# olegroshka/vae-channel-dynamics

Measured on AMD Instinct MI355X. Metric: images/sec SDXL-VAE train step @256x256 (tracking on), higher is better.
Workload: dtype f32

## Files before the change

### vae-channel-dynamics_amd/csrc/igemm.hip

```cpp
#include "bf16_frag.h"
#include <algorithm>
#include <stdlib.h>
#include <type_traits>

#include "launchers.h"

namespace {

struct LanePos {
  int lr, lh, trq, trp, trh;
};
__device__ __forceinline__ LanePos lane_pos(int lane) { return LanePos{lane & 31, lane >> 5, (lane & 15) >> 2, lane & 3, (lane >> 4) & 1}; }

struct F32 {
  typedef float elem;
  typedef f32x4 raw4;
  typedef f32x4 frag;
  typedef unsigned off_t;
  static constexpr int BK_ROWS = 32, BK_WGRAD = 32;
  static constexpr int KG = 8;
  static constexpr int PAD_K = 4, PAD_T = 4;
  static constexpr bool SETPRIO = true;
  static constexpr bool PAIR16 = false;
  static constexpr bool flag(int32_t) { return false; }
// ... 506 lines not shown
      if (XF != VAE_XF_NONE) {
        const bool ok = xb[i] >= 0;
        const int o = ok ? (xb[i] - b_lo) * BN + b4 * 4 : 0;
        v = xform4_tab<XF>(v, sS + o, sS + SS_HALF + o, ok);
      }
      P::put4(&sB[(bkq + BKR * i) * LDB + b4 * 4], v);
    }
  };
  typename P::frag fa[2][MI], fb[2][NI];
  auto fetch = [&](const elem* sA, const elem* sB, int kg, typename P::frag* a, typename P::frag* b) {
    P::template frags_tt<MI, NI>(a, b, sA, LDA, wm * TM, sB, LDB, wn * TN, kg, lp);
  };
  constexpr int NKG = BK / P::KG;
  auto compute = [&](const elem* sA, const elem* sB, int kg) {
    if (kg + 1 < NKG) fetch(sA, sB, kg + 1, fa[(kg + 1) & 1], fb[(kg + 1) & 1]);
    __builtin_amdgcn_sched_barrier(0);
    if (P::SETPRIO) __builtin_amdgcn_s_setprio(1);
    P::mma(acc, fa[kg & 1], fb[kg & 1]);
    if (P::SETPRIO) __builtin_amdgcn_s_setprio(0);
    __builtin_amdgcn_sched_barrier(0);
  };
  if (steps > 0) {
    load_regs(0);
    __syncthreads();
    store_lds(smem, smem + SA);
    if (steps > 1) load_regs(1);
    __syncthreads();
    for (int s = 0; s < steps; ++s) {
      const elem* cA = smem + (s & 1) * STAGE;
      const elem* cB = cA + SA;
      fetch(cA, cB, 0, fa[0], fb[0]);
      compute(cA, cB, 0);
      if (NKG == 4) compute(cA, cB, 1);
      if (s + 1 < steps) {
        elem* nA = smem + ((s + 1) & 1) * STAGE;
        store_lds(nA, nA + SA);
        if (s + 2 < steps) load_regs(s + 2);
      }
      compute(cA, cB, NKG / 2);
      if (NKG == 4) compute(cA, cB, 3);
      __syncthreads();
    }
  }

  const int64_t ld = (int64_t)g.taps * p.N;
  float* __restrict__ O = (p.nsplit == 1 ? p.out : p.partial + (int64_t)split * p.M * ld) + (int64_t)z * p.sOb;
#pragma unroll
  for (int ni = 0; ni < NI; ++ni) {
    const int col = n0 + wn * TN + ni * 32 + lr;
    if (col >= p.N) continue;
#pragma unroll
    for (int mi = 0; mi < MI; ++mi)
#pragma unroll
      for (int r = 0; r < 16; ++r) {
        const int row = m0 + wm * TM + mi * 32 + (r & 3) + 8 * (r >> 2) + 4 * lh;
        if (row < p.M) O[(int64_t)row * ld + (int64_t)tap * p.N + col] = p.alpha * acc[mi][ni][r];
      }
  }
  if (do_bias) {
    f32x4* red = reinterpret_cast<f32x4*>(smem);
    red[akq * AQ + a4] = bsum;
    __syncthreads();
    if (tid < AQ) {
      f32x4 t = {0.f, 0.f, 0.f, 0.f};
      for (int r = 0; r < AKR; ++r) t += red[r * AQ + tid];
#pragma unroll
      for (int e = 0; e < 4; ++e) {
        const int m = m0 + tid * 4 + e;
        if (m < p.M) p.bias_partial[(int64_t)split * p.M + m] = t[e];
      }
    }
  }
}

template <int BM, int BN, int WM, int WN, bool BKM, bool VEC, int XF>
__global__ __launch_bounds__(64 * WM * WN) void igemm_rows_kernel(vae_igemm_args p) { rows_body<F32, BM, BN, WM, WN, BKM, VEC, XF>(p); }
template <int BM, int BN, int WM, int WN, bool VEC, int XF>
__global__ __launch_bounds__(64 * WM * WN) void wgrad_kernel(vae_wgrad_args p) { wgrad_body<F32, BM, BN, WM, WN, VEC, XF>(p); }
template <int BM, int BN, int WM, int WN, bool BKM, int XF>
__global__ __launch_bounds__(64 * WM * WN) void igemm_rows_bf16_kernel(vae_igemm_args p) { rows_body<BF16, BM, BN, WM, WN, BKM, true, XF>(p); }
template <int BM, int BN, int WM, int WN, int XF>
__global__ __launch_bounds__(64 * WM * WN) void wgrad_bf16_kernel(vae_wgrad_args p) { wgrad_body<BF16, BM, BN, WM, WN, true, XF>(p); }

template <int KP>
__global__ __launch_bounds__(256) void reduce_splits_kernel(const float* __restrict__ partial, int nsplit, int64_t n, float* __restrict__ out,
                                                            int main_blocks, const float* __restrict__ partial2, int n2, float* __restrict__ out2) {
  constexpr int COLS = 256 / KP;
  __shared__ f32x4 red[KP > 1 ? 256 : 1];
  if ((int)blockIdx.x >= main_blocks) {
    const int i = ((int)blockIdx.x - main_blocks) * 256 + threadIdx.x;
    if (i < n2) {
      float s2 = 0.f;
      for (int k = 0; k < nsplit; ++k) s2 += partial2[(int64_t)k * n2 + i];
      out2[i] = s2;
    }
    return;
  }
  const int col = threadIdx.x % COLS, kp = threadIdx.x / COLS;
  const int64_t n4 = n >> 2;
  const int per = (nsplit + KP - 1) / KP;
  const int k0 = kp * per, k1 = min(nsplit, k0 + per);
  auto column = [&](int64_t i) {
    f32x4 s = {0.f, 0.f, 0.f, 0.f};
    const f32x4* p = reinterpret_cast<const f32x4*>(partial) + i;
    int k = k0;
    for (; k + 8 <= k1; k += 8) {
      f32x4 v[8];
#pragma unroll
      for (int j = 0; j < 8; ++j) v[j] = p[(int64_t)(k + j) * n4];
      s += ((v[0] + v[1]) + (v[2] + v[3])) + ((v[4] + v[5]) + (v[6] + v[7]));
    }
    for (; k < k1; ++k) s += p[(int64_t)k * n4];
    return s;
  };
  if (KP == 1) {
    for (int64_t i = (int64_t)blockIdx.x * 256 + threadIdx.x; i < n4; i += (int64_t)main_blocks * 256) reinterpret_cast<f32x4*>(out)[i] = column(i);
    return;
  }
  const int64_t i = (int64_t)blockIdx.x * COLS + col;
  f32x4 s = {0.f, 0.f, 0.f, 0.f};
  if (i < n4) s = column(i);
  red[threadIdx.x] = s;
  __syncthreads();
  if (kp == 0 && i < n4) {
#pragma unroll
    for (int j = 1; j < KP; ++j) s += red[j * COLS + col];
    reinterpret_cast<f32x4*>(out)[i] = s;
  }
}
__global__ void reduce_splits_scalar_kernel(const float* __restrict__ partial, int nsplit, int64_t n, float* __restrict__ out) {
  int64_t i = (int64_t)blockIdx.x * blockDim.x + threadIdx.x;
  const int64_t stride = (int64_t)gridDim.x * blockDim.x;
  for (; i < n; i += stride) {
    float s = 0.f;
    for (int k = 0; k < nsplit; ++k) s += partial[(int64_t)k * n + i];
    out[i] = s;
  }
}

template <int V>
using int_c = std::integral_constant<int, V>;
using std::false_type;
using std::true_type;

template <class Launch>
bool dispatch_xf(int xf, Launch launch) {
  switch (xf) {
    case VAE_XF_NONE: launch(int_c<VAE_XF_NONE>{}); return true;
    case VAE_XF_AFFINE: launch(int_c<VAE_XF_AFFINE>{}); return true;
    case VAE_XF_AFFINE_SILU: launch(int_c<VAE_XF_AFFINE_SILU>{}); return true;
    default: return false;
  }
}

template <bool BF, int BM, int BN, int WM, int WN>
int launch_rows_tile(const vae_igemm_args& a, bool bkm, bool vec, hipStream_t st) {
  const dim3 grid((unsigned)(((a.M + BM - 1) / BM) * ((a.N + BN - 1) / BN)), 1, (unsigned)a.batch), block(64 * WM * WN);
  auto go = [&](auto bkm_c, auto vec_c) {
    constexpr bool BKM = decltype(bkm_c)::value, VEC = decltype(vec_c)::value;
    auto launch = [&](auto xf) {
      if constexpr (BF) hipLaunchKernelGGL((igemm_rows_bf16_kernel<BM, BN, WM, WN, BKM, decltype(xf)::value>), grid, block, 0, st, a);
      else hipLaunchKernelGGL((igemm_rows_kernel<BM, BN, WM, WN, BKM, VEC, decltype(xf)::value>), grid, block, 0, st, a);
    };
    if constexpr (BKM) {
      if (a.xf != VAE_XF_NONE) { vae_set_error("igemm_rows: xf unsupported with n-contiguous weights"); return VAE_EINVAL; }
      launch(int_c<VAE_XF_NONE>{});
    } else if (!dispatch_xf(a.xf, launch)) {
      vae_set_error("igemm_rows: bad xf %d", a.xf);
      return VAE_EINVAL;
    }
    return 0;
  };
  if (BF || vec) return bkm ? go(true_type{}, true_type{}) : go(false_type{}, true_type{});
  if constexpr (!BF) return bkm ? go(true_type{}, false_type{}) : go(false_type{}, false_type{});
  return 0;
}
template <bool BF>
int launch_rows(const vae_igemm_args& a, bool bkm, bool vec, hipStream_t st) {
  return (a.N <= 32) ? launch_rows_tile<BF, 128, 32, 4, 1>(a, bkm, vec, st) : launch_rows_tile<BF, 128, 128, 4, 2>(a, bkm, vec, st);
}

template <bool BF, int BM, int BN, int WM, int WN>
int launch_wgrad_tile(const vae_wgrad_args& a, bool vec, hipStream_t st) {
  const dim3 grid((unsigned)(((a.M + BM - 1) / BM) * ((a.N + BN - 1) / BN)), (unsigned)(a.g.taps * a.nsplit), (unsigned)a.batch), block(64 * WM * WN);
  auto go = [&](auto vec_c) {
    auto launch = [&](auto xf) {
      if constexpr (BF) hipLaunchKernelGGL((wgrad_bf16_kernel<BM, BN, WM, WN, decltype(xf)::value>), grid, block, 0, st, a);
      else hipLaunchKernelGGL((wgrad_kernel<BM, BN, WM, WN, decltype(vec_c)::value, decltype(xf)::value>), grid, block, 0, st, a);
    };
    if (dispatch_xf(a.xf, launch)) return 0;
    vae_set_error("wgrad: bad xf %d", a.xf);
    return VAE_EINVAL;
  };
  if (BF || vec) return go(true_type{});
  if constexpr (!BF) return go(false_type{});
  return 0;
}
template <bool BF>
int launch_wgrad(const vae_wgrad_args& a, bool vec, hipStream_t st) {
  if (a.M <= 32) return launch_wgrad_tile<BF, 32, 128, 1, 4>(a, vec, st);
  if (a.N <= 32) return launch_wgrad_tile<BF, 128, 32, 4, 1>(a, vec, st);
  return launch_wgrad_tile<BF, 128, 128, 4, 2>(a, vec, st);
}

}

int launch_rows_f32(const vae_igemm_args& a, bool bkm, bool vec, hipStream_t st) { return launch_rows<false>(a, bkm, vec, st); }
int launch_rows_bf16(const vae_igemm_args& a, bool bkm, hipStream_t st) { return launch_rows<true>(a, bkm, true, st); }
int launch_wgrad_f32(const vae_wgrad_args& a, bool vec, hipStream_t st) { return launch_wgrad<false>(a, vec, st); }
int launch_wgrad_bf16(const vae_wgrad_args& a, hipStream_t st) { return launch_wgrad<true>(a, true, st); }

static int reduce_splits_impl(const float* partial, int32_t nsplit, int64_t n, float* out, const float* partial2, int32_t n2, float* out2,
                              hipStream_t st) {
  const int extra = partial2 ? (n2 + 255) / 256 : 0;
  if (n % 4 == 0 && aligned16(partial) && aligned16(out)) {
    const int64_t n4 = n / 4;
    if (nsplit >= 32) {
      const int64_t blocks = (n4 + 63) / 64;
      VAE_CHECK(blocks + extra < (1ll << 31), "reduce_splits: too many elements");
      hipLaunchKernelGGL(reduce_splits_kernel<4>, dim3((unsigned)(blocks + extra)), dim3(256), 0, st, partial, nsplit, n, out, (int)blocks, partial2, n2, out2);
    } else {
      const int64_t blocks = std::min<int64_t>((n4 + 255) / 256, 8192);
      hipLaunchKernelGGL(reduce_splits_kernel<1>, dim3((unsigned)(blocks + extra)), dim3(256), 0, st, partial, nsplit, n, out, (int)blocks, partial2, n2, out2);
    }
  } else {
    int blocks = (int)((n + 255) / 256);
    if (blocks > 4096) blocks = 4096;
    hipLaunchKernelGGL(reduce_splits_scalar_kernel, dim3(blocks), dim3(256), 0, st, partial, nsplit, n, out);
    if (partial2) hipLaunchKernelGGL(reduce_splits_scalar_kernel, dim3(extra), dim3(256), 0, st, partial2, nsplit, (int64_t)n2, out2);
  }
  return 0;
}
extern "C" int vae_reduce_splits(const float* partial, int32_t nsplit, int64_t n, float* out, void* stream) {
  VAE_CHECK(partial && out && nsplit > 0 && n > 0, "reduce_splits: bad args");
  if (int rc = reduce_splits_impl(partial, nsplit, n, out, nullptr, 0, nullptr, (hipStream_t)stream)) return rc;
  VAE_LAUNCH_CHECK("reduce_splits");
  return VAE_OK;
}
extern "C" int vae_reduce_splits2(const float* partial, int32_t nsplit, int64_t n, float* out, const float* partial2, int32_t n2, float* out2,
                                  void* stream) {
  VAE_CHECK(partial && out && partial2 && out2 && nsplit > 0 && n > 0 && n2 > 0, "reduce_splits2: bad args");
  if (int rc = reduce_splits_impl(partial, nsplit, n, out, partial2, n2, out2, (hipStream_t)stream)) return rc;
  VAE_LAUNCH_CHECK("reduce_splits2");
  return VAE_OK;
}
extern "C" int vae_wgrad_wino_reduce(const float* slab, int32_t nsplit, int32_t npos, int32_t Cin, int32_t Cout, float* scratch, float* dW,
                                     const float* bias_partial, float* db, void* stream) {
  VAE_CHECK(slab && dW && nsplit > 0 && Cin > 0 && Cout > 0 && Cin % 32 == 0 && Cout % 32 == 0, "wgrad_wino_reduce: bad args");
  VAE_CHECK(npos == 16 || npos == 9, "wgrad_wino_reduce: npos must be 16 (plain 3x3 layer) or 9 (upsampler convolution)");
  VAE_CHECK((bias_partial == nullptr) == (db == nullptr), "wgrad_wino_reduce: bias_partial and db go together");
  VAE_CHECK(nsplit == 1 || scratch != nullptr, "wgrad_wino_reduce: nsplit > 1 needs the [16*Cin*Cout] scratch buffer");
  hipStream_t st = (hipStream_t)stream;
  if (nsplit > 1) {
    if (int rc = reduce_splits_impl(slab, nsplit, (int64_t)npos * Cin * Cout, scratch, bias_partial, bias_partial ? Cout : 0, db, st)) return rc;
    VAE_LAUNCH_CHECK("reduce_splits");
    if (int rc = (npos == 9 ? launch_upwino_wgrad_reduce : launch_wino_wgrad_reduce)(scratch, 1, Cin, Cout, dW, nullptr, nullptr, st)) return rc;
  } else {
    if (int rc = (npos == 9 ? launch_upwino_wgrad_reduce : launch_wino_wgrad_reduce)(slab, 1, Cin, Cout, dW, bias_partial, db, st)) return rc;
  }
  VAE_LAUNCH_CHECK("wino_wgrad_reduce");
  return VAE_OK;
}
```

### vae-channel-dynamics_amd/csrc/launchers.h

```cpp
#pragma once
#include "common_host.h"

int launch_rows_f32(const vae_igemm_args& a, bool bkm, bool vec, hipStream_t st);
int launch_wgrad_f32(const vae_wgrad_args& a, bool vec, hipStream_t st);
int launch_rows_bf16(const vae_igemm_args& a, bool bkm, hipStream_t st);
int launch_wgrad_bf16(const vae_wgrad_args& a, hipStream_t st);

bool conv3_tile_eligible(const vae_igemm_args& a, bool vec, bool bkm);
int conv3_tile_gstat_chunks(const vae_igemm_args& a);
int launch_conv3_tile(const vae_igemm_args& a, bool bkm, hipStream_t st);
bool conv3_tile_bf16_packed(const vae_igemm_args& a);
int conv3_tile_bf16_gstat_chunks(const vae_igemm_args& a);
int launch_conv3_tile_bf16(const vae_igemm_args& a, bool bkm, hipStream_t st);
bool conv3_wide_bf16_eligible(const vae_igemm_args& a);
int conv3_wide_bf16_gstat_chunks(const vae_igemm_args& a);
int launch_conv3_wide_bf16(const vae_igemm_args& a, hipStream_t st);
bool conv3_wino_eligible(const vae_igemm_args& a);
int conv3_wino_nb();
int conv3_wino_gstat_chunks(const vae_igemm_args& a);
int conv3_wino_gnb_chunks(const vae_igemm_args& a);
int launch_wino_weights(const vae_igemm_args& a, float* U, hipStream_t st);
int launch_conv3_wino(const vae_igemm_args& a, const float* U, hipStream_t st);
bool conv3_wino4_eligible(const vae_igemm_args& a);
int conv3_wino4_gstat_chunks(const vae_igemm_args& a);
int conv3_wino4_gnb_chunks(const vae_igemm_args& a);
int launch_wino4_weights(const vae_igemm_args& a, float* U, hipStream_t st);
int launch_conv3_wino4(const vae_igemm_args& a, const float* U, hipStream_t st);
bool conv3_upwino_eligible(const vae_igemm_args& a);
int launch_upwino_weights(const vae_igemm_args& a, float* U, hipStream_t st);
int launch_conv3_upwino(const vae_igemm_args& a, const float* U, hipStream_t st);
bool conv1_bf16_eligible(const vae_igemm_args& a);
int launch_conv1_bf16(const vae_igemm_args& a, hipStream_t st);
bool conv_smallk_eligible(const vae_igemm_args& a);
int launch_conv_smallk(const vae_igemm_args& a, hipStream_t st);
bool conv_smalln_eligible(const vae_igemm_args& a);
int launch_conv_smalln(const vae_igemm_args& a, hipStream_t st);
bool conv_thin_bf16_eligible(const vae_igemm_args& a);
int launch_conv_thin_bf16(const vae_igemm_args& a, hipStream_t st);
bool conv_thinn_bf16_eligible(const vae_igemm_args& a);
int launch_conv_thinn_bf16(const vae_igemm_args& a, hipStream_t st);
int wgrad_smallk_kind(const vae_wgrad_args& a);
int wgrad_smallk_tiles(const vae_wgrad_args& a);
int launch_wgrad_smallk(const vae_wgrad_args& a, hipStream_t st);
bool wgrad_thin_bf16_eligible(const vae_wgrad_args& a, int kind);
int launch_wgrad_thin(const vae_wgrad_args& a, hipStream_t st);

bool wgrad3_tile_eligible(const vae_wgrad_args& a, bool vec);
int64_t wgrad3_tile_units(const vae_conv_geom& g);
int launch_wgrad3_tile(const vae_wgrad_args& a, hipStream_t st);
bool wgrad3_dma_bf16_operands(const vae_wgrad_args& a);
bool wgrad3_tile_bf16_eligible(const vae_wgrad_args& a, bool vec, bool dma);
int64_t wgrad3_tile_bf16_units(const vae_conv_geom& g);
int wgrad3_tile_bf16_columns(const vae_wgrad_args& a);
int launch_wgrad3_tile_bf16(const vae_wgrad_args& a, hipStream_t st);
int launch_wgrad3_dma_bf16(const vae_wgrad_args& a, hipStream_t st);
bool wgrad3_wino_eligible(const vae_wgrad_args& a);
int64_t wgrad3_wino_units(const vae_conv_geom& g);
int launch_wgrad3_wino(const vae_wgrad_args& a, hipStream_t st);
int launch_wino_wgrad_reduce(const float* slab, int nsplit, int N, int M, float* dW, const float* bpart, float* db, hipStream_t st);
bool wgrad3_upwino_eligible(const vae_wgrad_args& a);
int64_t wgrad3_upwino_units(const vae_conv_geom& g);
int launch_wgrad3_upwino(const vae_wgrad_args& a, hipStream_t st);
int launch_upwino_wgrad_reduce(const float* slab, int nsplit, int N, int M, float* dW, const float* bpart, float* db, hipStream_t st);
```

### vae-channel-dynamics_amd/csrc/wgrad3_upwino.hip

```cpp
#include "common.h"
#include <algorithm>
#include <type_traits>

namespace {

constexpr int GCI = 32, GCO = 128, NPOS = 9, GNT = 512, GNB = GCO / 32;
constexpr int XSX = 12;
constexpr int XSY = 20;
constexpr int SXF = 3 * GCI * XSX;
constexpr int SYF = 2 * GCO * XSY;
constexpr int GSTAGE = SXF + SYF;

__global__ __launch_bounds__(GNT, 2) void wgrad3_upwino_kernel(vae_wgrad_args p, int strips, int64_t nunits) {
  __shared__ __attribute__((aligned(16))) float smem[2 * GSTAGE];

  const int tid = threadIdx.x, lane = tid & 63, wave = tid >> 6;
  const int lr = lane & 31, lh = lane >> 5;
  const vae_conv_geom g = p.g;
  const int tilesN = p.N / GCI, ntile = tilesN * (p.M / GCO);
  int tile, split;
  {
    const int L = blockIdx.x, ns = p.nsplit;
    if (ns % 8 == 0) {
      const int j = L >> 3;
// ... 113 lines not shown
  using I2 = std::integral_constant<int, 2>;

  auto run = [&](auto PR, auto PC, auto EXTRA) {
    constexpr bool extra = decltype(EXTRA)::value;
    auto step = [&](int k, const Stg& cur, Stg& nxt) {
      const float* cx = smem + (k & 1) * GSTAGE;
      const float* cy = cx + SXF;
      float* nst = smem + ((k + 1) & 1) * GSTAGE;
      f32x4 a4, bb[2];
      build_a(PR, PC, cx, a4);
      build_b(PR, PC, cy, 0, bb[0]);
#pragma unroll
      for (int nb = 0; nb < GNB; ++nb) {
        __builtin_amdgcn_sched_barrier(0);
        if (nb == 1) {
          load_unit(k + 2, nxt);
          __builtin_amdgcn_sched_barrier(0);
        }
        if (nb + 1 < GNB) build_b(PR, PC, cy, nb + 1, bb[(nb + 1) & 1]);
#pragma unroll
        for (int e = 0; e < 4; ++e) acc[nb] = __builtin_amdgcn_mfma_f32_32x32x2f32(a4[e], bb[nb & 1][e], acc[nb], 0, 0, 0);
        __builtin_amdgcn_sched_barrier(0);
      }
      if (extra) {
        f32x4 ax, bx;
        build_a(I2{}, I2{}, cx, ax);
        build_b(I2{}, I2{}, cy, wave, bx);
#pragma unroll
        for (int e = 0; e < 4; ++e) accx = __builtin_amdgcn_mfma_f32_32x32x2f32(ax[e], bx[e], accx, 0, 0, 0);
      }
      store_unit(nst, cur);
      __syncthreads();
    };
    int k = 0;
    for (; k + 1 < nu; k += 2) {
      step(k, s1, s0);
      step(k + 1, s0, s1);
    }
    if (k < nu) step(k, s1, s0);
  };
  {
    using I0 = std::integral_constant<int, 0>;
    using I1 = std::integral_constant<int, 1>;
    using T = std::true_type;
    using F_ = std::false_type;
    switch (wave) {
      case 0: run(I0{}, I0{}, T{}); break;
      case 1: run(I0{}, I1{}, T{}); break;
      case 2: run(I0{}, I2{}, T{}); break;
      case 3: run(I1{}, I0{}, T{}); break;
      case 4: run(I1{}, I1{}, F_{}); break;
      case 5: run(I1{}, I2{}, F_{}); break;
      case 6: run(I2{}, I0{}, F_{}); break;
      default: run(I2{}, I1{}, F_{}); break;
    }
  }

  float* __restrict__ O = p.partial + (int64_t)split * NPOS * p.N * p.M;
#pragma unroll
  for (int nb = 0; nb < GNB; ++nb)
#pragma unroll
    for (int e = 0; e < 16; ++e) {
      const int ci = n0 + (e & 3) + 8 * (e >> 2) + 4 * lh;
      O[((int64_t)wave * p.N + ci) * p.M + m0 + nb * 32 + lr] = acc[nb][e];
    }
  if (wave < 4) {
#pragma unroll
    for (int e = 0; e < 16; ++e) {
      const int ci = n0 + (e & 3) + 8 * (e >> 2) + 4 * lh;
      O[((int64_t)8 * p.N + ci) * p.M + m0 + wave * 32 + lr] = accx[e];
    }
  }
  if (do_bias) {
#pragma unroll
    for (int e = 0; e < 4; ++e) {
      float sv = bsum[e];
#pragma unroll
      for (int o = 1; o < 16; o <<= 1) sv += __shfl_xor(sv, o, 64);
      if (xx == 0) p.bias_partial[(int64_t)split * p.M + m0 + 4 * yq + e] = sv;
    }
  }
}

__global__ __launch_bounds__(256) void upwino_wgrad_reduce_kernel(const float* __restrict__ slab, int nsplit, int N, int M, float* __restrict__ dW,
                                                                  int tiles, const float* __restrict__ bpart, float* __restrict__ db) {
  __shared__ float sT[9][32][33];
  const int tid = threadIdx.x;
  if ((int)blockIdx.x >= tiles) {
    const int m = ((int)blockIdx.x - tiles) * 256 + tid;
    if (m < M) {
      float s = 0.f;
      for (int k = 0; k < nsplit; ++k) s += bpart[(int64_t)k * M + m];
      db[m] = s;
    }
    return;
  }
  const int tilesM = M / 32;
  const int c0 = ((int)blockIdx.x / tilesM) * 32, m0 = ((int)blockIdx.x % tilesM) * 32;
  const int64_t pstride = (int64_t)N * M, sstride = NPOS * pstride;
#pragma unroll 1
  for (int r = 0; r < 4; ++r) {
    const int cl = (tid >> 5) + 8 * r, ml = tid & 31;
    const float* src = slab + (int64_t)(c0 + cl) * M + m0 + ml;
    float mm[9];
#pragma unroll
    for (int q = 0; q < 9; ++q) {
      float s = 0.f;
      for (int k = 0; k < nsplit; ++k) s += src[(int64_t)k * sstride + q * pstride];
      mm[q] = s;
    }
    float h[3][3];
#pragma unroll
    for (int j = 0; j < 3; ++j) {
      h[0][j] = mm[0 * 3 + j] + mm[1 * 3 + j];
      h[1][j] = mm[1 * 3 + j];
      h[2][j] = mm[1 * 3 + j] - mm[2 * 3 + j];
    }
#pragma unroll
    for (int a = 0; a < 3; ++a) {
      sT[a * 3 + 0][ml][cl] = h[a][0] + h[a][1];
      sT[a * 3 + 1][ml][cl] = h[a][1];
      sT[a * 3 + 2][ml][cl] = h[a][1] - h[a][2];
    }
  }
  __syncthreads();
#pragma unroll 1
  for (int r = 0; r < 4; ++r) {
    const int ml = (tid >> 5) + 8 * r, cl = tid & 31;
#pragma unroll
    for (int t = 0; t < 9; ++t) dW[((int64_t)(m0 + ml) * 9 + t) * N + c0 + cl] = sT[t][ml][cl];
  }
}

}

bool wgrad3_upwino_eligible(const vae_wgrad_args& a) {
  const vae_conv_geom& g = a.g;
  if (a.prec != VAE_PREC_F32 || a.X16 != nullptr || a.dY16 != nullptr || a.dY == nullptr || a.batch != 1 || a.alpha != 1.0f) return false;
  if (a.x_bf16 || a.y_bf16 || a.xf != VAE_XF_NONE) return false;
  if (g.taps != 9 || g.stride != 1 || g.pad_t != 1 || g.pad_l != 1 || g.mode != VAE_MODE_UP2X) return false;
  if (a.tapmask != 0 || a.y_step > 1 || g.Ho != 2 * g.Hs || g.Wo != 2 * g.Ws) return false;
  if (g.Ws % 8 != 0 || a.N % GCI != 0 || a.M % GCO != 0 || g.Cs % 4 != 0 || a.ldy % 4 != 0 || g.Cs < a.N) return false;
  if (!aligned16(a.X) || !aligned16(a.dY)) return false;
  if ((size_t)g.B * g.Hs * g.Ws * g.Cs * 4u >= BUF_MAX || (size_t)g.B * g.Ho * g.Wo * a.ldy * 4u >= BUF_MAX) return false;
  return true;
}

int64_t wgrad3_upwino_units(const vae_conv_geom& g) { return (int64_t)g.B * g.Hs * (g.Ws / 8); }

int launch_wgrad3_upwino(const vae_wgrad_args& a, hipStream_t st) {
  const vae_conv_geom& g = a.g;
  const int64_t nunits = wgrad3_upwino_units(g);
  dim3 grid((unsigned)((a.M / GCO) * (a.N / GCI) * a.nsplit), 1, 1);
  hipLaunchKernelGGL(wgrad3_upwino_kernel, grid, dim3(GNT), 0, st, a, g.Ws / 8, nunits);
  return 0;
}

int launch_upwino_wgrad_reduce(const float* slab, int nsplit, int N, int M, float* dW, const float* bpart, float* db, hipStream_t st) {
  const int tiles = (N / 32) * (M / 32);
  const int extra = bpart ? (M + 255) / 256 : 0;
  hipLaunchKernelGGL(upwino_wgrad_reduce_kernel, dim3((unsigned)(tiles + extra)), dim3(256), 0, st, slab, nsplit, N, M, dW, tiles, bpart, db);
  return 0;
}
```

### vae-channel-dynamics_amd/csrc/wgrad3_wino.hip

```cpp
#include "common.h"
#ifndef VAE_ABLATE
#define VAE_ABLATE 0
#endif
#include <algorithm>
#include <type_traits>

namespace {

constexpr int GCI = 32, GCO = 128, GNT = 512;
constexpr int XS = 20;
constexpr int SXF = 4 * GCI * XS;
constexpr int SYF = 2 * GCO * XS;
constexpr int GSTAGE = SXF + SYF;

template <int XF>
__global__ __launch_bounds__(GNT, 1) void wgrad3_wino_kernel(vae_wgrad_args p, int strips, int64_t nunits) {
  __shared__ __attribute__((aligned(16))) float smem[2 * GSTAGE];

  const int tid = threadIdx.x, lane = tid & 63, wave = tid >> 6;
  const int lr = lane & 31, lh = lane >> 5;
  const vae_conv_geom g = p.g;
  const int tilesN = p.N / GCI, ntile = tilesN * (p.M / GCO);
  int tile, split;
  {
// ... 169 lines not shown
            a4[1][e] = rc[2 * e + 1] + rc[2 * e + 2];
          } else {
            a4[0][e] = rc[2 * e + 2] - rc[2 * e + 1];
            a4[1][e] = rc[2 * e + 1] - rc[2 * e + 3];
          }
        }
        build_b(rd, bb[0]);
        read_d(1, rd);
      }
      if (!(VAE_ABLATE & 2) && wave < 4) store_unit(nst, cur);
#pragma unroll
      for (int nb = 0; nb < 4; ++nb) {
        __builtin_amdgcn_sched_barrier(0);
        if (nb == 1) {
          if (!(VAE_ABLATE & 1)) load_unit(k + 2, nxt);
          __builtin_amdgcn_sched_barrier(0);
        }
        if (nb == 3 && wave >= 4) {
          if (!(VAE_ABLATE & 2)) store_unit(nst, cur);
          __builtin_amdgcn_sched_barrier(0);
        }
        if (nb < 3) build_b(rd, bb[(nb + 1) & 1]);
        if (nb < 2) read_d(nb + 2, rd);
#pragma unroll
        for (int pi = 0; pi < 2; ++pi)
#pragma unroll
          for (int e = 0; e < 4; ++e) acc[pi][nb] = __builtin_amdgcn_mfma_f32_32x32x2f32(a4[pi][e], bb[nb & 1][pi][e], acc[pi][nb], 0, 0, 0);
#pragma unroll
        for (int i = 0; i < 4; ++i) {
          __builtin_amdgcn_sched_group_barrier(0x008, 1, 0);
          __builtin_amdgcn_sched_group_barrier(0x002, 3, 0);
        }
        __builtin_amdgcn_sched_group_barrier(0x100, 4, 0);
        __builtin_amdgcn_sched_group_barrier(0x008, 4, 0);
        __builtin_amdgcn_sched_barrier(0);
      }
      if (!(VAE_ABLATE & 16)) __syncthreads();
    };
    int k = 0;
    for (; k + 1 < nu; k += 2) {
      step(k, s1, s0);
      step(k + 1, s0, s1);
    }
    if (k < nu) step(k, s1, s0);
  };
  {
    using J0 = std::integral_constant<int, 0>;
    using J1 = std::integral_constant<int, 1>;
    switch (wave) {
      case 0: run(std::integral_constant<int, 0>{}, J0{}); break;
      case 1: run(std::integral_constant<int, 0>{}, J1{}); break;
      case 2: run(std::integral_constant<int, 1>{}, J0{}); break;
      case 3: run(std::integral_constant<int, 1>{}, J1{}); break;
      case 4: run(std::integral_constant<int, 2>{}, J0{}); break;
      case 5: run(std::integral_constant<int, 2>{}, J1{}); break;
      case 6: run(std::integral_constant<int, 3>{}, J0{}); break;
      default: run(std::integral_constant<int, 3>{}, J1{}); break;
    }
  }

  float* __restrict__ O = p.partial + (int64_t)split * 16 * p.N * p.M;
#pragma unroll
  for (int pi = 0; pi < 2; ++pi) {
    const int pos = wi * 4 + 2 * jh + pi;
#pragma unroll
    for (int nb = 0; nb < 4; ++nb)
#pragma unroll
      for (int e = 0; e < 16; ++e) {
        const int ci = n0 + (e & 3) + 8 * (e >> 2) + 4 * lh;
        O[((int64_t)pos * p.N + ci) * p.M + m0 + nb * 32 + lr] = acc[pi][nb][e];
      }
  }
  if (do_bias) {
#pragma unroll
    for (int e = 0; e < 4; ++e) {
      float s = bsum[e];
#pragma unroll
      for (int o = 1; o < 16; o <<= 1) s += __shfl_xor(s, o, 64);
      if (xx == 0) p.bias_partial[(int64_t)split * p.M + m0 + 4 * yq + e] = s;
    }
  }
}

__global__ __launch_bounds__(256) void wino_wgrad_reduce_kernel(const float* __restrict__ slab, int nsplit, int N, int M, float* __restrict__ dW,
                                                                int tiles, const float* __restrict__ bpart, float* __restrict__ db) {
  __shared__ float sT[9][32][33];
  const int tid = threadIdx.x;
  if ((int)blockIdx.x >= tiles) {
    const int m = ((int)blockIdx.x - tiles) * 256 + tid;
    if (m < M) {
      float s = 0.f;
      for (int k = 0; k < nsplit; ++k) s += bpart[(int64_t)k * M + m];
      db[m] = s;
    }
    return;
  }
  const int tilesM = M / 32;
  const int c0 = ((int)blockIdx.x / tilesM) * 32, m0 = ((int)blockIdx.x % tilesM) * 32;
  const int64_t pstride = (int64_t)N * M, sstride = 16 * pstride;
#pragma unroll 1
  for (int r = 0; r < 4; ++r) {
    const int cl = (tid >> 5) + 8 * r, ml = tid & 31;
    const float* src = slab + (int64_t)(c0 + cl) * M + m0 + ml;
    float mm[16];
#pragma unroll
    for (int q = 0; q < 16; ++q) {
      float s = 0.f;
      for (int k = 0; k < nsplit; ++k) s += src[(int64_t)k * sstride + q * pstride];
      const float ci = ((q >> 2) == 1 || (q >> 2) == 2) ? 0.5f : 1.f, cj = ((q & 3) == 1 || (q & 3) == 2) ? 0.5f : 1.f;
      mm[q] = s * (ci * cj);
    }
    float h[3][4];
#pragma unroll
    for (int j = 0; j < 4; ++j) {
      h[0][j] = (mm[0 * 4 + j] + mm[1 * 4 + j]) + mm[2 * 4 + j];
      h[1][j] = mm[1 * 4 + j] - mm[2 * 4 + j];
      h[2][j] = (mm[1 * 4 + j] + mm[2 * 4 + j]) - mm[3 * 4 + j];
    }
#pragma unroll
    for (int a = 0; a < 3; ++a) {
      sT[a * 3 + 0][ml][cl] = (h[a][0] + h[a][1]) + h[a][2];
      sT[a * 3 + 1][ml][cl] = h[a][1] - h[a][2];
      sT[a * 3 + 2][ml][cl] = (h[a][1] + h[a][2]) - h[a][3];
    }
  }
  __syncthreads();
#pragma unroll 1
  for (int r = 0; r < 4; ++r) {
    const int ml = (tid >> 5) + 8 * r, cl = tid & 31;
#pragma unroll
    for (int t = 0; t < 9; ++t) dW[((int64_t)(m0 + ml) * 9 + t) * N + c0 + cl] = sT[t][ml][cl];
  }
}

}

bool wgrad3_wino_eligible(const vae_wgrad_args& a) {
  const vae_conv_geom& g = a.g;
  if (a.prec != VAE_PREC_F32 || a.X16 != nullptr || a.dY16 != nullptr || a.dY == nullptr || a.batch != 1 || a.alpha != 1.0f) return false;
  if (g.taps != 9 || g.stride != 1 || g.pad_t != 1 || g.pad_l != 1 || g.mode != VAE_MODE_FWD) return false;
  if (a.tapmask != 0 || a.y_step > 1 || g.Ho != g.Hs || g.Wo != g.Ws) return false;
  if (g.Ho % 2 != 0 || g.Wo % 16 != 0 || a.N % GCI != 0 || a.M % GCO != 0 || g.Cs % 4 != 0 || a.ldy % 4 != 0) return false;
  if (!aligned16(a.X) || !aligned16(a.dY)) return false;
  if ((size_t)g.B * g.Hs * g.Ws * g.Cs * 4u >= BUF_MAX || (size_t)g.B * g.Ho * g.Wo * a.ldy * 4u >= BUF_MAX) return false;
  return true;
}

int64_t wgrad3_wino_units(const vae_conv_geom& g) { return (int64_t)g.B * (g.Ho / 2) * (g.Wo / 16); }

int launch_wgrad3_wino(const vae_wgrad_args& a, hipStream_t st) {
  const vae_conv_geom& g = a.g;
  const int64_t nunits = wgrad3_wino_units(g);
  dim3 grid((unsigned)((a.M / GCO) * (a.N / GCI) * a.nsplit), 1, 1);
  const int strips = g.Wo / 16;
  if (a.xf == VAE_XF_NONE) hipLaunchKernelGGL(wgrad3_wino_kernel<VAE_XF_NONE>, grid, dim3(GNT), 0, st, a, strips, nunits);
  else if (a.xf == VAE_XF_AFFINE) hipLaunchKernelGGL(wgrad3_wino_kernel<VAE_XF_AFFINE>, grid, dim3(GNT), 0, st, a, strips, nunits);
  else hipLaunchKernelGGL(wgrad3_wino_kernel<VAE_XF_AFFINE_SILU>, grid, dim3(GNT), 0, st, a, strips, nunits);
  return 0;
}

int launch_wino_wgrad_reduce(const float* slab, int nsplit, int N, int M, float* dW, const float* bpart, float* db, hipStream_t st) {
  const int tiles = (N / 32) * (M / 32);
  const int extra = bpart ? (M + 255) / 256 : 0;
  hipLaunchKernelGGL(wino_wgrad_reduce_kernel, dim3((unsigned)(tiles + extra)), dim3(256), 0, st, slab, nsplit, N, M, dW, tiles, bpart, db);
  return 0;
}
```

### vae-channel-dynamics_amd/src/vaehip/ops.py

```python
from __future__ import annotations

import ctypes as C
import os
from typing import NamedTuple, Optional, Tuple

import torch

from .lib import ConvGeom, IgemmArgs, WgradArgs, lib

XF_NONE, XF_AFFINE, XF_AFFINE_SILU = 0, 1, 2
PREC_F32, PREC_BF16 = 0, 1
PRECISION = PREC_F32

WEIGHTS16: Optional[Tuple[int, int, int]] = None


def pack_bf16(src: torch.Tensor, dst: torch.Tensor) -> torch.Tensor:
    assert src.is_contiguous() and dst.is_contiguous() and dst.numel() == src.numel() and dst.element_size() == 2
    lib.call("vae_pack_bf16", _p(src), src.numel(), _p(dst), _stream())
    return dst


def _wh(w: torch.Tensor):
    if PRECISION != PREC_BF16 or WEIGHTS16 is None:
# ... 545 lines not shown
    a.C = _p(out)
    wu = _wino_weights(a, dev) if wino else None
    if gnb is not None and not pool and gnb.x.shape == out.shape and not (want16 and out.dtype != torch.bfloat16):
        a.gnb_x, a.gnb_x_bf16 = _p(gnb.x), _b16(gnb.x)
        a.gnb_mean, a.gnb_rstd, a.gnb_gamma, a.gnb_beta = _p(gnb.st.mean), _p(gnb.st.rstd), _p(gnb.gamma), _p(gnb.beta)
        a.gnb_groups, a.gnb_silu = int(gnb.groups), int(gnb.silu)
        nch = lib.query("vae_conv_gnb_chunks", C.byref(a))
        if nch > 0:
            ws = torch.empty((B, nch, Ci, 2), device=dev, dtype=torch.float32)
            a.gnb_ws = _p(ws)
            out._gnb = (ws, nch, _gnb_key(gnb.x, gnb.st, gnb.gamma, gnb.beta, gnb.silu))
        else:
            a.gnb_x = None
    _launch_igemm(a)
    if pool:
        pooled = torch.empty((B, H, W, Ci), device=dev, dtype=torch.float32)
        lib.call("vae_sumpool2x2", _p(out), B, H, W, Ci, _p(pooled), _stream())
        out = pooled
    if want16 and out.dtype != torch.bfloat16:
        return to_bf16(out)
    return out


def _upconv_phase_wgrad(dy, x, gv, bgrad_out, dy16=None) -> bool:
    Co, _, _, Ci = gv.shape
    B, H, W, Cs = x.shape
    if Cs != Ci:
        return False
    xb = x.dtype == torch.bfloat16
    a = wgrad_phase_args(B, H, W, Co, Ci)
    a.dY, a.X = _p(dy if dy is not None else dy16), _p(x)
    if not lib.query("vae_wgrad_phase_ok", C.byref(a)):
        return False
    images = PRECISION == PREC_BF16 and Cs % 8 == 0 and Co % 8 == 0
    x16 = None
    if images:
        x16 = x if xb else getattr(x, "_b16", None)
        a.X16 = _p(x16) if x16 is not None else _UNALLOCATED
        a.dY16 = _p(dy16) if dy16 is not None else _UNALLOCATED
    elif xb or dy is None:
        return False
    ns, fus = C.c_int32(0), C.c_int32(0)
    lib.call("vae_wgrad_plan", C.byref(a), C.byref(ns), C.byref(fus))
    ns = ns.value
    a.nsplit = ns
    if images:
        if x16 is None:
            x16 = pack_bf16(x, torch.empty(x.shape, device=x.device, dtype=torch.bfloat16))
        if dy16 is None:
            dy16 = pack_bf16(dy, torch.empty(dy.shape, device=dy.device, dtype=torch.bfloat16))
            dy._b16 = dy16
        a.X16, a.dY16 = _p(x16), _p(dy16)
    n = Co * 9 * Ci
    dwe = torch.empty((4, n), device=x.device, dtype=torch.float32)
    dbe = torch.empty((4, Co), device=x.device, dtype=torch.float32) if bgrad_out is not None else None
    partial = torch.empty((ns, n), device=x.device, dtype=torch.float32) if ns > 1 else None
    bpart = torch.empty((ns, Co), device=x.device, dtype=torch.float32) if bgrad_out is not None else None
    a.partial, a.bias_partial = _p(partial), _p(bpart)
    for ph, a.tapmask, a.y_oy, a.y_ox, _, _ in _phases():
        a.out = _p(dwe[ph]) if ns == 1 else None
        _launch_wgrad(a)
        _reduce_splits(partial, bpart, ns, n, Co, dwe[ph], None if dbe is None else dbe[ph])
    lib.call("vae_upconv_fold_wgrad", _p(dwe), _p(dbe), Co, Ci, _p(gv), _p(bgrad_out), _stream())
    return True


def _wgrad_wino(a: WgradArgs, gv: torch.Tensor, bgrad_out: Optional[torch.Tensor], dev) -> bool:
    if not WINOGRAD or PRECISION != PREC_F32:
        return False
    ns = C.c_int32(0)
    lib.call("vae_wgrad_wino_plan", C.byref(a), C.byref(ns))
    ns = ns.value
    if ns <= 0:
        return False
    npos = int(lib.query("vae_wgrad_wino_positions", C.byref(a)))
    slab = torch.empty((ns, npos * a.N * a.M), device=dev, dtype=torch.float32)
    bpart = torch.empty((ns, a.M), device=dev, dtype=torch.float32) if bgrad_out is not None else None
    a.nsplit, a.partial, a.bias_partial = ns, _p(slab), _p(bpart)
    fl = 2.0 * a.M * a.N * a.npix * 9
    if npos == 9:
        _timed("wgrad3_upwino_kernel", fl, fl * 0.25, "vae_wgrad_wino", C.byref(a), _stream())
    else:
        _timed(f"wgrad3_wino_kernel<{a.xf}>", fl, fl * WINO_EXECUTED, "vae_wgrad_wino", C.byref(a), _stream())
    scratch = torch.empty((npos * a.N * a.M,), device=dev, dtype=torch.float32) if ns > 1 else None
    _timed("wgrad_wino_reduce (split sum + output transform)", 0.0, 0.0, "vae_wgrad_wino_reduce", _p(slab), ns, npos, a.N, a.M,
           _p(scratch), _p(gv), _p(bpart), _p(bgrad_out), _stream())
    return True


def conv_wgrad(dy: torch.Tensor, x: torch.Tensor, kind: str, wgrad_out: torch.Tensor,
               bgrad_out: Optional[torch.Tensor], *, xf: int = XF_NONE, stats: Optional[Stats] = None,
               x16: Optional[torch.Tensor] = None):
    dy16 = _grad16(dy)
    dy32 = dy if dy.dtype == torch.float32 else None
    _chk_act(dy, "conv_wgrad.dy")
    _chk_act(x, "conv_wgrad.x")
    if x16 is not None:
        assert x16.shape == x.shape and x16.dtype == torch.bfloat16 and x16.is_contiguous()
        xf = XF_NONE
    gv = ohwi(wgrad_out)
    Co, _, _, Ci = gv.shape
    B, H, W, Cs = x.shape
    assert dy.shape == (B, *out_hw(kind, H, W), Co), (dy.shape, kind, x.shape, Co)
    if (kind == "c3up" and PRECISION == PREC_F32 and WINOGRAD and xf == XF_NONE and x16 is None and dy32 is not None
            and x.dtype == torch.float32):
        a = wgrad_args(kind, B, H, W, Cs, Co, Ci)
        a.dY, a.X = _p(dy32), _p(x)
        if _wgrad_wino(a, gv, bgrad_out, x.device):
            return
    if kind == "c3up" and PHASE_UPCONV and xf == XF_NONE and x16 is None and _upconv_phase_wgrad(dy32, x, gv, bgrad_out, dy16):
        return
    xb = x.dtype == torch.bfloat16
    use16 = dy16 is not None and (dy32 is None or grad_image_ok(kind, x.shape, Co, Ci))
    a = wgrad_args(kind, B, H, W, Cs, Co, Ci, xf=xf)
    a.dY, a.X = _p(dy32 if dy32 is not None else dy16), _p(x)
    a.dY16 = _p(dy16) if use16 else None
    if x16 is not None:
        a.X16 = _p(x16)
    elif xb and xf == XF_NONE:
        a.X16 = _p(x)
    elif xb:
        a.x_bf16 = 1
    if xf != XF_NONE:
        assert stats is not None
        a.scale, a.shift = _p(stats.scale), _p(stats.shift)
    if _wgrad_wino(a, gv, bgrad_out, x.device):
        return
    ns, fus = C.c_int32(0), C.c_int32(0)
    lib.call("vae_wgrad_plan", C.byref(a), C.byref(ns), C.byref(fus))
    if xf != XF_NONE and not fus.value:
        x, xf = gn_apply(x, stats, xf), XF_NONE
        a.X, a.xf, a.scale, a.shift, a.x_bf16 = _p(x), XF_NONE, None, None, 0
        lib.call("vae_wgrad_plan", C.byref(a), C.byref(ns), C.byref(fus))
    if (a.X16 or a.dY16 or a.x_bf16) and not lib.query("vae_wgrad_io16_ok", C.byref(a)):
        x32 = to_f32(x16) if x16 is not None else to_f32(x)
        return conv_wgrad(dy32 if dy32 is not None else to_f32(dy16), x32, kind, wgrad_out, bgrad_out, xf=xf, stats=stats)
    ns = ns.value
    a.nsplit = ns
    partial = None
    if ns == 1:
        a.out = _p(gv)
    else:
        partial = torch.empty((ns, gv.numel()), device=x.device, dtype=torch.float32)
        a.partial = _p(partial)
    bpart = None
    if bgrad_out is not None:
        bpart = torch.empty((ns, Co), device=x.device, dtype=torch.float32)
        a.bias_partial = _p(bpart)
    _launch_wgrad(a)
    _reduce_splits(partial, bpart, ns, gv.numel(), Co, gv, bgrad_out)


_GN_TARGET = 1024


def _gn_nchunk(B: int, HW: int, Cc: int) -> int:
    pr = max(1, 256 // (Cc // 4))
    return max(1, min(_GN_TARGET // max(B, 1), HW // (16 * pr) if HW >= 16 * pr else 1))


def gn_stats(x: torch.Tensor, gamma: torch.Tensor, beta: torch.Tensor, G: int = GN_GROUPS, eps: float = GN_EPS) -> Stats:
    _chk_act(x, "gn_stats.x")
    B, H, W, Cc = x.shape
    HW = H * W
    dev = x.device
    fused = getattr(x, "_gstat", None)
    if fused is not None and fused[1] == G:
        ws, nch = fused[0], fused[2]
    else:
# ... 290 lines not shown
```

Baseline: 103.4.

## Fuse Winograd wgrad split reduction with output transform in one vectorized kernel

The split sum over the Winograd weight-gradient slab and the inverse output transform used to run as two kernels when nsplit > 1, with a scratch buffer in between. They now run as a single templated kernel that reads the slab with f32x4 loads, splits positions and split ranges across threads, and reduces through shared memory. The tile width along Cin is chosen from the channel counts so small layers still fill the GPU, and the bias column sums are unrolled. This removes a kernel launch and the scratch write and read, in exchange for more complex indexing and more shared-memory use per block.

```diff
diff --git a/vae-channel-dynamics_amd/csrc/igemm.hip b/vae-channel-dynamics_amd/csrc/igemm.hip
--- a/vae-channel-dynamics_amd/csrc/igemm.hip
+++ b/vae-channel-dynamics_amd/csrc/igemm.hip
@@ -612,18 +612,30 @@
 template <int BM, int BN, int WM, int WN, int XF>
 __global__ __launch_bounds__(64 * WM * WN) void wgrad_bf16_kernel(vae_wgrad_args p) { wgrad_body<BF16, BM, BN, WM, WN, true, XF>(p); }
 
+__device__ __forceinline__ void small_column_sums(const float* __restrict__ partial2, int nsplit, int n2, float* __restrict__ out2, int blk) {
+  const int i = blk * 256 + (int)threadIdx.x;
+  if (i >= n2) return;
+  const float* p = partial2 + i;
+  float s = 0.f;
+  int k = 0;
+  for (; k + 16 <= nsplit; k += 16) {
+    float v[16];
+#pragma unroll
+    for (int j = 0; j < 16; ++j) v[j] = p[(int64_t)(k + j) * n2];
+#pragma unroll
+    for (int j = 0; j < 16; ++j) s += v[j];
+  }
+  for (; k < nsplit; ++k) s += p[(int64_t)k * n2];
+  out2[i] = s;
+}
+
 template <int KP>
 __global__ __launch_bounds__(256) void reduce_splits_kernel(const float* __restrict__ partial, int nsplit, int64_t n, float* __restrict__ out,
                                                             int main_blocks, const float* __restrict__ partial2, int n2, float* __restrict__ out2) {
   constexpr int COLS = 256 / KP;
   __shared__ f32x4 red[KP > 1 ? 256 : 1];
   if ((int)blockIdx.x >= main_blocks) {
-    const int i = ((int)blockIdx.x - main_blocks) * 256 + threadIdx.x;
-    if (i < n2) {
-      float s2 = 0.f;
-      for (int k = 0; k < nsplit; ++k) s2 += partial2[(int64_t)k * n2 + i];
-      out2[i] = s2;
-    }
+    small_column_sums(partial2, nsplit, n2, out2, (int)blockIdx.x - main_blocks);
     return;
   }
   const int col = threadIdx.x % COLS, kp = threadIdx.x / COLS;
@@ -665,6 +677,132 @@
     float s = 0.f;
     for (int k = 0; k < nsplit; ++k) s += partial[(int64_t)k * n + i];
     out[i] = s;
+  }
+}
+
+template <int NPOS, int TCI>
+__global__ __launch_bounds__(256) void wgrad_wino_reduce_kernel(const float* __restrict__ slab, int nsplit, int N, int M, float* __restrict__ dW,
+                                                                int tiles, const float* __restrict__ bpart, float* __restrict__ db) {
+  constexpr int TQ = 8, TCO = 4 * TQ, Q = TCI * TQ, KP = 256 / Q, NP = (NPOS + KP - 1) / KP;
+  constexpr int ST0 = KP > 1 ? NPOS * Q * 4 : 0;
+  __shared__ __attribute__((aligned(16))) float smem[ST0 + 9 * TCO * (TCI + 1)];
+  const int tid = threadIdx.x;
+  if ((int)blockIdx.x >= tiles) {
+    small_column_sums(bpart, nsplit, M, db, (int)blockIdx.x - tiles);
+    return;
+  }
+  const int tilesM = M / TCO;
+  const int c0 = ((int)blockIdx.x / tilesM) * TCI, m0 = ((int)blockIdx.x % tilesM) * TCO;
+  const int q = tid % Q, kp = tid / Q;
+  const int cq = q % TQ, cl = q / TQ;
+  const int64_t pstride4 = ((int64_t)N * M) >> 2, sstride4 = NPOS * pstride4;
+  const f32x4* src = reinterpret_cast<const f32x4*>(slab + (int64_t)(c0 + cl) * M + m0 + 4 * cq);
+  const f32x4* sp[NP];
+#pragma unroll
+  for (int j = 0; j < NP; ++j) sp[j] = src + (kp + j * KP < NPOS ? kp + j * KP : 0) * pstride4;
+  auto tree8 = [](const f32x4* v) { return ((v[0] + v[1]) + (v[2] + v[3])) + ((v[4] + v[5]) + (v[6] + v[7])); };
+  auto range = [&](int k0, int k1, f32x4(&g)[NP]) {
+#pragma unroll
+    for (int j = 0; j < NP; ++j) g[j] = f32x4{0.f, 0.f, 0.f, 0.f};
+    int k = k0;
+    if constexpr (NP == 1) {
+      for (; k + 16 <= k1; k += 16) {
+        f32x4 v[16];
+#pragma unroll
+        for (int i = 0; i < 16; ++i) v[i] = sp[0][(int64_t)(k + i) * sstride4];
+        g[0] += tree8(v);
+        g[0] += tree8(v + 8);
+      }
+    }
+    for (; k + 8 <= k1; k += 8) {
+#pragma unroll
+      for (int j = 0; j < NP; ++j) {
+        f32x4 v[8];
+#pragma unroll
+        for (int i = 0; i < 8; ++i) v[i] = sp[j][(int64_t)(k + i) * sstride4];
+        g[j] += tree8(v);
+      }
+    }
+    for (; k < k1; ++k) {
+      f32x4 v[NP];
+#pragma unroll
+      for (int j = 0; j < NP; ++j) v[j] = sp[j][(int64_t)k * sstride4];
+#pragma unroll
+      for (int j = 0; j < NP; ++j) g[j] += v[j];
+    }
+  };
+  f32x4 mine[NP];
+  if (nsplit >= 32) {
+    const int per = (nsplit + 3) / 4;
+    range(0, min(nsplit, per), mine);
+    for (int r = 1; r < 4; ++r) {
+      f32x4 g[NP];
+      range(r * per, min(nsplit, (r + 1) * per), g);
+#pragma unroll
+      for (int j = 0; j < NP; ++j) mine[j] += g[j];
+    }
+  } else {
+    range(0, nsplit, mine);
+  }
+  f32x4 acc[NPOS];
+  if constexpr (KP > 1) {
+    f32x4* red = reinterpret_cast<f32x4*>(smem);
+#pragma unroll
+    for (int j = 0; j < NP; ++j)
+      if (kp + j * KP < NPOS) red[(kp + j * KP) * Q + q] = mine[j];
+    __syncthreads();
+    if (kp == 0) {
+#pragma unroll
+      for (int p = 0; p < NPOS; ++p) acc[p] = red[p * Q + q];
+    }
+  } else {
+#pragma unroll
+    for (int p = 0; p < NPOS; ++p) acc[p] = mine[p];
+  }
+  float(*sT)[TCO][TCI + 1] = reinterpret_cast<float(*)[TCO][TCI + 1]>(smem + ST0);
+  if (kp == 0) {
+    f32x4 o[9];
+    if constexpr (NPOS == 16) {
+      f32x4 h[3][4];
+#pragma unroll
+      for (int j = 0; j < 4; ++j) {
+        const float cj = (j == 1 || j == 2) ? 0.5f : 1.f;
+        const f32x4 r0 = acc[0 * 4 + j] * cj, r1 = acc[1 * 4 + j] * (0.5f * cj), r2 = acc[2 * 4 + j] * (0.5f * cj), r3 = acc[3 * 4 + j] * cj;
+        h[0][j] = (r0 + r1) + r2;
+        h[1][j] = r1 - r2;
+        h[2][j] = (r1 + r2) - r3;
+      }
+#pragma unroll
+      for (int a = 0; a < 3; ++a) {
+        o[a * 3 + 0] = (h[a][0] + h[a][1]) + h[a][2];
+        o[a * 3 + 1] = h[a][1] - h[a][2];
+        o[a * 3 + 2] = (h[a][1] + h[a][2]) - h[a][3];
+      }
+    } else {
+      f32x4 h[3][3];
+#pragma unroll
+      for (int j = 0; j < 3; ++j) {
+        h[0][j] = acc[0 * 3 + j] + acc[1 * 3 + j];
+        h[1][j] = acc[1 * 3 + j];
+        h[2][j] = acc[1 * 3 + j] - acc[2 * 3 + j];
+      }
+#pragma unroll
+      for (int a = 0; a < 3; ++a) {
+        o[a * 3 + 0] = h[a][0] + h[a][1];
+        o[a * 3 + 1] = h[a][1];
+        o[a * 3 + 2] = h[a][1] - h[a][2];
+      }
+    }
+#pragma unroll
+    for (int t = 0; t < 9; ++t)
+#pragma unroll
+      for (int e = 0; e < 4; ++e) sT[t][4 * cq + e][cl] = o[t][e];
+  }
+  __syncthreads();
+  for (int idx = tid; idx < 9 * TCO * TCI; idx += 256) {
+    const int c = idx % TCI, r = idx / TCI;
+    const int t = r % 9, ml = r / 9;
+    dW[((int64_t)(m0 + ml) * 9 + t) * N + c0 + c] = sT[t][ml][c];
   }
 }
 
@@ -779,15 +917,25 @@
   VAE_CHECK(slab && dW && nsplit > 0 && Cin > 0 && Cout > 0 && Cin % 32 == 0 && Cout % 32 == 0, "wgrad_wino_reduce: bad args");
   VAE_CHECK(npos == 16 || npos == 9, "wgrad_wino_reduce: npos must be 16 (plain 3x3 layer) or 9 (upsampler convolution)");
   VAE_CHECK((bias_partial == nullptr) == (db == nullptr), "wgrad_wino_reduce: bias_partial and db go together");
-  VAE_CHECK(nsplit == 1 || scratch != nullptr, "wgrad_wino_reduce: nsplit > 1 needs the [16*Cin*Cout] scratch buffer");
+  VAE_CHECK(aligned16(slab), "wgrad_wino_reduce: the slab must be 16-byte aligned");
+  VAE_CHECK((int64_t)Cin * Cout <= (1ll << 30), "wgrad_wino_reduce: too many channel pairs");
+  (void)scratch;
   hipStream_t st = (hipStream_t)stream;
-  if (nsplit > 1) {
-    if (int rc = reduce_splits_impl(slab, nsplit, (int64_t)npos * Cin * Cout, scratch, bias_partial, bias_partial ? Cout : 0, db, st)) return rc;
-    VAE_LAUNCH_CHECK("reduce_splits");
-    if (int rc = (npos == 9 ? launch_upwino_wgrad_reduce : launch_wino_wgrad_reduce)(scratch, 1, Cin, Cout, dW, nullptr, nullptr, st)) return rc;
-  } else {
-    if (int rc = (npos == 9 ? launch_upwino_wgrad_reduce : launch_wino_wgrad_reduce)(slab, 1, Cin, Cout, dW, bias_partial, db, st)) return rc;
-  }
-  VAE_LAUNCH_CHECK("wino_wgrad_reduce");
+  const int extra = bias_partial ? (Cout + 255) / 256 : 0;
+  auto launch = [&](auto npos_c, auto tci_c) {
+    constexpr int NPOS = decltype(npos_c)::value, TCI = decltype(tci_c)::value;
+    const int tiles = (Cin / TCI) * (Cout / 32);
+    hipLaunchKernelGGL((wgrad_wino_reduce_kernel<NPOS, TCI>), dim3((unsigned)(tiles + extra)), dim3(256), 0, st, slab, nsplit, Cin, Cout, dW, tiles,
+                       bias_partial, db);
+  };
+  const int64_t t32 = (int64_t)(Cin / 32) * (Cout / 32);
+  auto pick = [&](auto npos_c) {
+    if (t32 >= 256) launch(npos_c, int_c<32>{});
+    else if (4 * t32 >= 256) launch(npos_c, int_c<8>{});
+    else launch(npos_c, int_c<2>{});
+  };
+  if (npos == 9) pick(int_c<9>{});
+  else pick(int_c<16>{});
+  VAE_LAUNCH_CHECK("wgrad_wino_reduce");
   return VAE_OK;
 }
diff --git a/vae-channel-dynamics_amd/csrc/launchers.h b/vae-channel-dynamics_amd/csrc/launchers.h
--- a/vae-channel-dynamics_amd/csrc/launchers.h
+++ b/vae-channel-dynamics_amd/csrc/launchers.h
@@ -57,8 +57,6 @@
 bool wgrad3_wino_eligible(const vae_wgrad_args& a);
 int64_t wgrad3_wino_units(const vae_conv_geom& g);
 int launch_wgrad3_wino(const vae_wgrad_args& a, hipStream_t st);
-int launch_wino_wgrad_reduce(const float* slab, int nsplit, int N, int M, float* dW, const float* bpart, float* db, hipStream_t st);
 bool wgrad3_upwino_eligible(const vae_wgrad_args& a);
 int64_t wgrad3_upwino_units(const vae_conv_geom& g);
 int launch_wgrad3_upwino(const vae_wgrad_args& a, hipStream_t st);
-int launch_upwino_wgrad_reduce(const float* slab, int nsplit, int N, int M, float* dW, const float* bpart, float* db, hipStream_t st);
diff --git a/vae-channel-dynamics_amd/csrc/wgrad3_upwino.hip b/vae-channel-dynamics_amd/csrc/wgrad3_upwino.hip
--- a/vae-channel-dynamics_amd/csrc/wgrad3_upwino.hip
+++ b/vae-channel-dynamics_amd/csrc/wgrad3_upwino.hip
@@ -219,56 +219,6 @@
   }
 }
 
-__global__ __launch_bounds__(256) void upwino_wgrad_reduce_kernel(const float* __restrict__ slab, int nsplit, int N, int M, float* __restrict__ dW,
-                                                                  int tiles, const float* __restrict__ bpart, float* __restrict__ db) {
-  __shared__ float sT[9][32][33];
-  const int tid = threadIdx.x;
-  if ((int)blockIdx.x >= tiles) {
-    const int m = ((int)blockIdx.x - tiles) * 256 + tid;
-    if (m < M) {
-      float s = 0.f;
-      for (int k = 0; k < nsplit; ++k) s += bpart[(int64_t)k * M + m];
-      db[m] = s;
-    }
-    return;
-  }
-  const int tilesM = M / 32;
-  const int c0 = ((int)blockIdx.x / tilesM) * 32, m0 = ((int)blockIdx.x % tilesM) * 32;
-  const int64_t pstride = (int64_t)N * M, sstride = NPOS * pstride;
-#pragma unroll 1
-  for (int r = 0; r < 4; ++r) {
-    const int cl = (tid >> 5) + 8 * r, ml = tid & 31;
-    const float* src = slab + (int64_t)(c0 + cl) * M + m0 + ml;
-    float mm[9];
-#pragma unroll
-    for (int q = 0; q < 9; ++q) {
-      float s = 0.f;
-      for (int k = 0; k < nsplit; ++k) s += src[(int64_t)k * sstride + q * pstride];
-      mm[q] = s;
-    }
-    float h[3][3];
-#pragma unroll
-    for (int j = 0; j < 3; ++j) {
-      h[0][j] = mm[0 * 3 + j] + mm[1 * 3 + j];
-      h[1][j] = mm[1 * 3 + j];
-      h[2][j] = mm[1 * 3 + j] - mm[2 * 3 + j];
-    }
-#pragma unroll
-    for (int a = 0; a < 3; ++a) {
-      sT[a * 3 + 0][ml][cl] = h[a][0] + h[a][1];
-      sT[a * 3 + 1][ml][cl] = h[a][1];
-      sT[a * 3 + 2][ml][cl] = h[a][1] - h[a][2];
-    }
-  }
-  __syncthreads();
-#pragma unroll 1
-  for (int r = 0; r < 4; ++r) {
-    const int ml = (tid >> 5) + 8 * r, cl = tid & 31;
-#pragma unroll
-    for (int t = 0; t < 9; ++t) dW[((int64_t)(m0 + ml) * 9 + t) * N + c0 + cl] = sT[t][ml][cl];
-  }
-}
-
 }
 
 bool wgrad3_upwino_eligible(const vae_wgrad_args& a) {
@@ -292,10 +242,3 @@
   hipLaunchKernelGGL(wgrad3_upwino_kernel, grid, dim3(GNT), 0, st, a, g.Ws / 8, nunits);
   return 0;
 }
-
-int launch_upwino_wgrad_reduce(const float* slab, int nsplit, int N, int M, float* dW, const float* bpart, float* db, hipStream_t st) {
-  const int tiles = (N / 32) * (M / 32);
-  const int extra = bpart ? (M + 255) / 256 : 0;
-  hipLaunchKernelGGL(upwino_wgrad_reduce_kernel, dim3((unsigned)(tiles + extra)), dim3(256), 0, st, slab, nsplit, N, M, dW, tiles, bpart, db);
-  return 0;
-}
diff --git a/vae-channel-dynamics_amd/csrc/wgrad3_wino.hip b/vae-channel-dynamics_amd/csrc/wgrad3_wino.hip
--- a/vae-channel-dynamics_amd/csrc/wgrad3_wino.hip
+++ b/vae-channel-dynamics_amd/csrc/wgrad3_wino.hip
@@ -275,57 +275,6 @@
   }
 }
 
-__global__ __launch_bounds__(256) void wino_wgrad_reduce_kernel(const float* __restrict__ slab, int nsplit, int N, int M, float* __restrict__ dW,
-                                                                int tiles, const float* __restrict__ bpart, float* __restrict__ db) {
-  __shared__ float sT[9][32][33];
-  const int tid = threadIdx.x;
-  if ((int)blockIdx.x >= tiles) {
-    const int m = ((int)blockIdx.x - tiles) * 256 + tid;
-    if (m < M) {
-      float s = 0.f;
-      for (int k = 0; k < nsplit; ++k) s += bpart[(int64_t)k * M + m];
-      db[m] = s;
-    }
-    return;
-  }
-  const int tilesM = M / 32;
-  const int c0 = ((int)blockIdx.x / tilesM) * 32, m0 = ((int)blockIdx.x % tilesM) * 32;
-  const int64_t pstride = (int64_t)N * M, sstride = 16 * pstride;
-#pragma unroll 1
-  for (int r = 0; r < 4; ++r) {
-    const int cl = (tid >> 5) + 8 * r, ml = tid & 31;
-    const float* src = slab + (int64_t)(c0 + cl) * M + m0 + ml;
-    float mm[16];
-#pragma unroll
-    for (int q = 0; q < 16; ++q) {
-      float s = 0.f;
-      for (int k = 0; k < nsplit; ++k) s += src[(int64_t)k * sstride + q * pstride];
-      const float ci = ((q >> 2) == 1 || (q >> 2) == 2) ? 0.5f : 1.f, cj = ((q & 3) == 1 || (q & 3) == 2) ? 0.5f : 1.f;
-      mm[q] = s * (ci * cj);
-    }
-    float h[3][4];
-#pragma unroll
-    for (int j = 0; j < 4; ++j) {
-      h[0][j] = (mm[0 * 4 + j] + mm[1 * 4 + j]) + mm[2 * 4 + j];
-      h[1][j] = mm[1 * 4 + j] - mm[2 * 4 + j];
-      h[2][j] = (mm[1 * 4 + j] + mm[2 * 4 + j]) - mm[3 * 4 + j];
-    }
-#pragma unroll
-    for (int a = 0; a < 3; ++a) {
-      sT[a * 3 + 0][ml][cl] = (h[a][0] + h[a][1]) + h[a][2];
-      sT[a * 3 + 1][ml][cl] = h[a][1] - h[a][2];
-      sT[a * 3 + 2][ml][cl] = (h[a][1] + h[a][2]) - h[a][3];
-    }
-  }
-  __syncthreads();
-#pragma unroll 1
-  for (int r = 0; r < 4; ++r) {
-    const int ml = (tid >> 5) + 8 * r, cl = tid & 31;
-#pragma unroll
-    for (int t = 0; t < 9; ++t) dW[((int64_t)(m0 + ml) * 9 + t) * N + c0 + cl] = sT[t][ml][cl];
-  }
-}
-
 }
 
 bool wgrad3_wino_eligible(const vae_wgrad_args& a) {
@@ -351,10 +300,3 @@
   else hipLaunchKernelGGL(wgrad3_wino_kernel<VAE_XF_AFFINE_SILU>, grid, dim3(GNT), 0, st, a, strips, nunits);
   return 0;
 }
-
-int launch_wino_wgrad_reduce(const float* slab, int nsplit, int N, int M, float* dW, const float* bpart, float* db, hipStream_t st) {
-  const int tiles = (N / 32) * (M / 32);
-  const int extra = bpart ? (M + 255) / 256 : 0;
-  hipLaunchKernelGGL(wino_wgrad_reduce_kernel, dim3((unsigned)(tiles + extra)), dim3(256), 0, st, slab, nsplit, N, M, dW, tiles, bpart, db);
-  return 0;
-}
diff --git a/vae-channel-dynamics_amd/src/vaehip/ops.py b/vae-channel-dynamics_amd/src/vaehip/ops.py
--- a/vae-channel-dynamics_amd/src/vaehip/ops.py
+++ b/vae-channel-dynamics_amd/src/vaehip/ops.py
@@ -651,9 +651,8 @@
         _timed("wgrad3_upwino_kernel", fl, fl * 0.25, "vae_wgrad_wino", C.byref(a), _stream())
     else:
         _timed(f"wgrad3_wino_kernel<{a.xf}>", fl, fl * WINO_EXECUTED, "vae_wgrad_wino", C.byref(a), _stream())
-    scratch = torch.empty((npos * a.N * a.M,), device=dev, dtype=torch.float32) if ns > 1 else None
     _timed("wgrad_wino_reduce (split sum + output transform)", 0.0, 0.0, "vae_wgrad_wino_reduce", _p(slab), ns, npos, a.N, a.M,
-           _p(scratch), _p(gv), _p(bpart), _p(bgrad_out), _stream())
+           None, _p(gv), _p(bpart), _p(bgrad_out), _stream())
     return True
 
 
```

After: 104.5, median of 6. 1.01x the previous value.
